# darioShar/DLPM

Measured on AMD Instinct MI355X. Metric: samples/sec at T=1000 (CIFAR-10 32x32, alpha=1.7), higher is better.
Workload: dtype f32 (1x1 / stride-2 convolutions: fp32 operands split exactly into 3 bf16 planes, bf16 MFMA products, fp32 accumulate)

## Files before the change

dlpm_amd/csrc/conv.h:

```cpp
#pragma once
#include "common.h"

namespace dlpm {

struct ConvLaunch {
    const float *src0 = nullptr, *src1 = nullptr;
    int C0 = 0, C1 = 0;
    int B = 0, Hin = 0, Win = 0, Hout = 0, Wout = 0;
    int ks = 1, stride = 1, ups = 0;
    const float *w = nullptr;
    const float *w_frag = nullptr;
    const float *w_wino = nullptr;
    const float *w_wino4 = nullptr;
    const float *w_wino4_n64 = nullptr, *w_wino4_n32 = nullptr;
    const float *w_wino4sp = nullptr;
    const void *w_split = nullptr;
    const float *w_small = nullptr;
    const float *w_taps = nullptr;
    const float *w_hfused = nullptr;
    const float *bias = nullptr;
    const float *coefA = nullptr, *coefB = nullptr;
    int act_silu = 0;
    const float *res0 = nullptr, *res1 = nullptr;
    int R0 = 0;
    float *out = nullptr;
    int Cout = 0;
    int in_nchw = 0, out_nchw = 0;
    int gen = 0;
    int64_t dispatch_B = 0;
    int gemm = 0;
    int ksplit = 0;
    float2 *stats_out = nullptr;
#ifdef DLPM_PHASE_TIMING
    unsigned long long *phase = nullptr;
#endif
};

bool igemm_supported(const ConvLaunch &c);

enum ConvFamily { CONV_HEAD_FUSED, CONV_HEAD_GEMM, CONV_HEAD, CONV_SPLIT, CONV_WINO4SP, CONV_WINO4, CONV_WINO, CONV_IGEMM, CONV_STEM, CONV_DIRECT };
struct ConvRoute {
    ConvFamily family = CONV_DIRECT;
    int bh = 0, bw = 0, nimg = 0;
    int nq = 0;
    int64_t grid = 0;
    int stats_px = 0;
    int ksplit = 1;
    int64_t scratch_floats = 0;
    char name[96] = "";
    bool head() const { return family <= CONV_HEAD; }
};
ConvRoute conv_route(const ConvLaunch &c);
struct HeadUpdate;
int launch_conv(const ConvLaunch &c, const HeadUpdate *hu, float *head_scratch, hipStream_t st);
int launch_conv_direct(const ConvLaunch &c, hipStream_t st);
int launch_conv_stem(const ConvLaunch &c, hipStream_t st);
struct HeadUpdate {
    float *x = nullptr;
    const float *z = nullptr;
// ... 21 lines not shown
int launch_conv_head_fused(const ConvLaunch &c, const HeadUpdate *hu, hipStream_t st);
bool wino_route(const ConvLaunch &c, ConvRoute *r);
int launch_conv_wino(const ConvLaunch &c, const ConvRoute &r, hipStream_t st);
int64_t wino_weight_floats(int Cout, int Cin);
int relayout_weight_wino(const float *oihw_dev, float *dst_dev, int Cout, int Cin, hipStream_t st);
bool wino4_enabled();
bool wino4_route(const ConvLaunch &c, ConvRoute *r);
int launch_conv_wino4(const ConvLaunch &c, const ConvRoute &r, hipStream_t st);
int64_t wino4_weight_floats(int Cout, int Cin);
int relayout_weight_wino4(const float *oihw_dev, float *dst_dev, int Cout, int Cin, hipStream_t st, int nq = 0);
bool wino4sp_enabled();
bool wino4sp_layer_ok(int Cout, int Cin, int Hlo, int Wlo);
int launch_conv_wino4sp(const ConvLaunch &c, const ConvRoute &r, hipStream_t st);
int64_t wino4sp_weight_floats(int Cout, int Cin);
int relayout_weight_wino4sp(const float *oihw_dev, float *dst_dev, int Cout, int Cin, hipStream_t st);
struct ResImgLaunch {
    const float *x0 = nullptr, *x1 = nullptr;
    int C0 = 0, C1 = 0, B = 0;
    int H = 32;
    const float2 *st0 = nullptr, *st1 = nullptr;
    int nt0 = 1, nt1 = 1;
    const float *coefA1 = nullptr, *coefB1 = nullptr;
    const float *gn1_w = nullptr, *gn1_b = nullptr, *gn2_w = nullptr, *gn2_b = nullptr;
    const float *w1 = nullptr, *b1 = nullptr;
    const float *w2 = nullptr, *b2 = nullptr;
    const float *emb = nullptr;
    int64_t emb_stride = 0;
    int emb_off = 0;
    const float *res = nullptr;
    float *hbuf = nullptr;
// ... 1 lines not shown
    float2 *stats_out = nullptr;
#ifdef DLPM_PHASE_TIMING
    unsigned long long *phase = nullptr;
#endif
};
bool res_img_ok(const ResImgLaunch &r);
int launch_resblock_img(const ResImgLaunch &r, hipStream_t st);

bool conv_split_ok(const ConvLaunch &c);
int launch_conv_split(const ConvLaunch &c, hipStream_t st);
int64_t split_weight_floats(int Cout, int Cin, int taps);
int relayout_weight_split(const float *oihw_dev, void *dst_dev, int Cout, int Cin, int taps, hipStream_t st);
constexpr int64_t NARROW_COPIES_MAX_BATCH = 512;
struct Conv3Layouts {
    bool frag = false, wino = false, wino4 = false, wino4sp = false;
    bool narrow = false;
};
bool wino4_narrow_copies_wanted(int Cout, int64_t dispatch_B);
Conv3Layouts conv3_layouts(const ConvLaunch &c);
int64_t splitk_partial_floats(const ConvLaunch &c, const ConvRoute &r);
int launch_conv_splitk(const ConvLaunch &c, const ConvRoute &r, float *part, hipStream_t st);
int launch_splitk_reduce(const float *part, int S, int64_t npix, int Cout, const float *bias, const float *res0, const float *res1, int R0,
                         float *out, hipStream_t st);
int relayout_weight(const float *oihw_dev, float *dst_dev, int Cout, int Cin, int ks, bool for_igemm, hipStream_t st);
int64_t frag_weight_floats(int Cout, int Cin);
int relayout_weight_frag(const float *oihw_dev, float *dst_dev, int Cout, int Cin, hipStream_t st);

int launch_gn_coeffs(const float *src0, const float *src1, int C0, int C1, int B, int HW, int groups,
                     const float *gamma, const float *beta, const float *ss, int64_t ss_stride, int64_t ss_offset,
                     float *coefA, float *coefB, hipStream_t st);
// ... 53 lines not shown
```

dlpm_amd/csrc/conv_igemm.hip:

```cpp
#include <cstdlib>

#include <algorithm>

#include "conv.h"
#include "igemm_epilogue.h"

namespace dlpm {
namespace {

constexpr int KC = 32;
constexpr int LDS_LD = 36;

template <int BN, int WAVES_M, int WAVES_N, int RM, int RN>
__device__ __forceinline__ void epilogue_rows(const ConvLaunch &p, floatx16 (&acc)[RM][RN], float *lds, int64_t m0, int n0,
                                              int64_t M, int tid, int wm, int wn, int l31, int kh) {
    constexpr int LD = BN + 4, PR = RM * 32, C4 = BN / 4, RG = 256 / C4;
    const int R1 = p.Cout - p.R0;
    const bool do_stats = p.stats_out != nullptr;
    float4 K = make_float4(0.f, 0.f, 0.f, 0.f), s1 = K, s2 = K;
    int cnt = 0;
    for (int ph = 0; ph < WAVES_M; ph++) {
        if (wm == ph) {
#pragma unroll
            for (int i = 0; i < RM; i++)
// ... 997 lines not shown
}

bool wino4_narrow_copies_wanted(int Cout, int64_t dispatch_B) {
    return Cout % 128 == 0 && dispatch_B > 0 && dispatch_B <= NARROW_COPIES_MAX_BATCH;
}

Conv3Layouts conv3_layouts(const ConvLaunch &c) {
    Conv3Layouts y;
    const int Cin = c.C0 + c.C1;
    const bool plain = !c.in_nchw && !c.out_nchw && c.stride == 1;
    if (!igemm_supported(c) || c.ks != 3 || Cin % 32 != 0) return y;
    y.frag = true;
    y.wino = plain && c.Cout % 64 == 0 && Cin % 16 == 0;
    y.wino4 = plain && wino4_enabled() && c.Cout % 32 == 0 && Cin % 8 == 0;
    y.wino4sp = y.wino4 && c.ups && wino4sp_layer_ok(c.Cout, Cin, c.Hin, c.Win);
    y.narrow = y.wino4 && wino4_narrow_copies_wanted(c.Cout, c.dispatch_B);
    return y;
}

ConvRoute conv_route(const ConvLaunch &c) {
    ConvRoute r;
    const int64_t hw = (int64_t)c.Hout * c.Wout;
    int th, nimg;
    const char *cls = nullptr;
    if (head_fused_ok(c)) {
        r.family = CONV_HEAD_FUSED;
    } else if (head_gemm_ok(c)) {
        r.family = CONV_HEAD_GEMM;
        r.scratch_floats = head_gemm_scratch_floats(c);
    } else if (head_conv_ok(c)) {
        r.family = CONV_HEAD;
    } else if (conv_split_ok(c)) {
        r.family = CONV_SPLIT;
        cls = c.ks == 1 ? "conv1x1_bf16x3" : "conv3x3_bf16x3";
        r.stats_px = (c.R0 & 3) ? 0 : hw % BM == 0 ? BM : hw == 64 ? 64 : 0;
    } else if (wino4_route(c, &r)) {
        cls = r.family == CONV_WINO4SP ? "conv3x3_wino4sp" : "conv3x3_wino4";
        if (r.family == CONV_WINO4 && r.nq != 128 && !(c.Cout == 32 && c.Hout == 32 && c.Wout == 32)) r.ksplit = ksplit_for(c, r.grid);
    } else if (!igemm_supported(c)) {
        r.family = conv_takes_stem(c) ? CONV_STEM : CONV_DIRECT;
        if (r.family == CONV_STEM && stem_stats_ok(c)) r.stats_px = 1024;
    } else if (wino_route(c, &r)) {
        cls = "conv3x3_wino";
        r.ksplit = ksplit_for(c, r.grid);
    } else {
        r.family = CONV_IGEMM;
        cls = c.ks == 3 ? (halo_ok(c, &th, &nimg) ? "conv3x3_halo" : "conv3x3_igemm") : "conv1x1_igemm";
        r.stats_px = (c.out_nchw || (c.Cout & 3) || (c.R0 & 3)) ? 0 : hw % BM == 0 ? BM : 0;
    }
    if (r.ksplit > 1) r.stats_px = 0;
    if (!cls) return r;
    if (prof_enabled() && prof_detail()) {
        const bool gemm = r.family == CONV_SPLIT || r.family == CONV_IGEMM;
// ... 107 lines not shown
```

dlpm_amd/csrc/conv_wino4.hip:

```cpp
#include <cstdlib>
#include <type_traits>

#include "conv.h"
#include "gn_stats.h"

namespace dlpm {
namespace {

typedef float floatx4 __attribute__((ext_vector_type(4)));

constexpr int F4_TILES = 16;
constexpr int F4_NQ = 128;
constexpr int F4_KC = 8;
constexpr int F4_RAWPIX = 576;
constexpr int F4_PRLD = F4_KC + 4;
constexpr int F4_NT = 512;
constexpr int F4_QNIT = (F4_RAWPIX * 2 + F4_NT - 1) / F4_NT;
constexpr int F4_RAWBUF = F4_RAWPIX * F4_PRLD + 16;
constexpr int F4_RAWPIX_N = 400;
constexpr int F4_RAWBUF_N = F4_RAWPIX_N * F4_PRLD + 16;
constexpr int f4_nq_of(int cout) { return cout % 128 == 0 ? 128 : cout % 64 == 0 ? 64 : 32; }
constexpr int F4_CFS = 16 * 2 * F4_KC;
constexpr int F4_VBUF = 36 * F4_TILES * F4_KC;
#ifndef F4_RING_DEPTH
// ... 1382 lines not shown
            F4_LDS_BARRIER();
            if (kh == 0 && lkv == 0) {
                const float2 a = part[chv], b = part[CO + chv];
                const float dd = b.x - a.x;
                p.stats_out[(int64_t)img * CO + chv] = make_float2(a.x + dd * 0.5f, a.y + b.y + dd * dd * 64.f);
            }
        }
    };
    if (kh == 0) epilogue(std::integral_constant<int, 0>());
    else epilogue(std::integral_constant<int, 2>());
    DLPM_PHASE(p, 10);
    DLPM_PHASE_FLUSH(p, 8);
#ifdef DLPM_PHASE_TIMING
    if (p.phase && tid == 0) atomicAdd(p.phase + 11, 1ull);
#endif
}

__global__ void k_relayout_weight_wino4(const float *oihw, float *dst, int Cout, int Cin, int nw) {
    const int nch = Cin / F4_KC;
    const int64_t total = (int64_t)Cout * Cin * 36;
    const int64_t i = (int64_t)blockIdx.x * blockDim.x + threadIdx.x;
    if (i >= total) return;
    const int e = (int)(i & 3);
    const int lane = (int)((i >> 2) & 63);
    int64_t r = i >> 8;
    const int pp = (int)(r % 18); r /= 18;
    const int chunk = (int)(r % nch); r /= nch;
    const int wave = (int)(r % nw);
    const int nt = (int)(r / nw);
    const int lk = lane >> 4, li = lane & 15;
// ... 109 lines not shown
    if (c.gen == DLPM_CONV_F2 || c.gen == DLPM_CONV_IGEMM) return false;
    if (!wino4_geometry_nq(c, nq, bh, bw, nimg)) return false;
    if (!c.w_wino || c.gen == DLPM_CONV_F4) return true;
    if (*nimg > 4) return false;
    if (c.dispatch_B <= 0) return true;
    return f4_mblocks(c.dispatch_B, c.Hout / 4, c.Wout / 4, *nimg) * (c.Cout / nq) >= 256;
}

static bool wino4_whole_image(const ConvLaunch &c) {
    static const int v = env_switch("DLPM_WINO4_IMG", 1);
    return v != 0 && c.Cout == 32 && !c.ups && c.Hout == 32 && c.Wout == 32 && (c.C0 + c.C1) <= 1024;
}

static int launch_conv_wino4_nq(const ConvLaunch &c, int nq, int bh, int bw, int nimg, hipStream_t st);

int launch_conv_wino4(const ConvLaunch &c, const ConvRoute &rt, hipStream_t st) {
    int bh, bw, nimg;
    if (rt.family != CONV_WINO4 || !wino4_geometry_nq(c, rt.nq, &bh, &bw, &nimg)) {
        set_error("launch_conv_wino4: unsupported shape");
        return DLPM_ERR_UNSUPPORTED;
    }
    const int nq = rt.nq;
    if (nq != f4_nq_of(c.Cout)) {
        ConvLaunch cn = c;
        cn.w_wino4 = nq == 64 ? c.w_wino4_n64 : c.w_wino4_n32;
        cn.w_wino4_n64 = cn.w_wino4_n32 = nullptr;
        cn.dispatch_B = 0;
        return launch_conv_wino4_nq(cn, nq, rt.bh, rt.bw, rt.nimg, st);
    }
    return launch_conv_wino4_nq(c, nq, rt.bh, rt.bw, rt.nimg, st);
}

// ... 103 lines not shown
    if (n * (4 * h + 1) * (4 * w + 1) > FS_RAWPIX) return false;
    *bh = h; *bw = w; *nimg = n;
    return true;
}
bool wino4sp_layer_ok(int Cout, int Cin, int Hlo, int Wlo) {
    int h, w, n;
    return wino4sp_enabled() && wino4sp_block(Cout, Cin, Hlo, Wlo, &h, &w, &n);
}

static bool wino4sp_geometry(const ConvLaunch &c, int *bh, int *bw, int *nimg) {
    if (!c.ups || !c.w_wino4sp || c.ks != 3 || c.stride != 1 || c.in_nchw || c.out_nchw) return false;
    if (c.Hout != 2 * c.Hin || c.Wout != 2 * c.Win || c.C0 % F4_KC != 0 || (c.R0 & 15) != 0 || c.ksplit > 1) return false;
    return wino4sp_block(c.Cout, c.C0 + c.C1, c.Hin, c.Win, bh, bw, nimg);
}

bool wino4_route(const ConvLaunch &c, ConvRoute *r) {
    const int nq = wino4_nq_for(c);
    int bh, bw, nimg;
    if (!wino4_preferred(c, nq, &bh, &bw, &nimg)) return false;
    r->family = CONV_WINO4;
    if (c.ups && c.w_wino4sp && wino4sp_enabled() && nq == F4_NQ && wino4sp_geometry(c, &bh, &bw, &nimg)) r->family = CONV_WINO4SP;
    else if (c.dispatch_B > 0) r->grid = f4_mblocks(c.dispatch_B, c.Hout / 4, c.Wout / 4, nimg) * (c.Cout / nq);
    r->bh = bh; r->bw = bw; r->nimg = nimg; r->nq = nq;
    r->stats_px = nimg == 1 ? 256 : (nimg == 4 && bh * bw == 4) ? 64 : 0;
    return true;
}

int launch_conv_wino4sp(const ConvLaunch &c, const ConvRoute &rt, hipStream_t st) {
    int bh, bw, nimg;
    if (rt.family != CONV_WINO4SP || !wino4sp_geometry(c, &bh, &bw, &nimg)) {
        set_error("launch_conv_wino4sp: unsupported shape");
// ... 23 lines not shown
```

dlpm_amd/csrc/unet.hip:

```cpp
#include <cmath>
#include <cstdlib>
#include <map>
#include <string>
#include <utility>
#include <vector>

#include "conv.h"
#include "../../include/dlpm_amd_chains.h"
#include "../../include/dlpm_amd_conv.h"

using namespace dlpm;

namespace {

struct Param {
    std::string key;
    int64_t numel = 0;
    float *dev = nullptr;
    bool set = false;
};

enum LayerKind { L_STEM, L_RES, L_ATTN, L_DOWN, L_UP };

struct ConvW {
    int p_w = -1, p_b = -1;
    int cout = 0, cin = 0, ks = 1;
    bool use_igemm = false;
    float *w_dev = nullptr;
    float *w_frag = nullptr;
    float *w_wino = nullptr;
    float *w_wino4 = nullptr;
    float *w_wino4_n64 = nullptr, *w_wino4_n32 = nullptr;
    float *w_wino4sp = nullptr;
    float *w_small = nullptr;
    float *w_taps = nullptr;
    float *w_split = nullptr;
    float *w_rs = nullptr;
    float *w_hfused = nullptr;
    bool owns = false;
};
constexpr float *ConvW::*OWNED_LAYOUTS[] = {&ConvW::w_frag, &ConvW::w_wino, &ConvW::w_wino4, &ConvW::w_wino4_n64, &ConvW::w_wino4_n32, &ConvW::w_wino4sp,
                                            &ConvW::w_small, &ConvW::w_taps, &ConvW::w_split, &ConvW::w_rs, &ConvW::w_hfused};
constexpr struct { int nq; float *ConvW::*copy; } NARROW_LAYOUTS[] = {{64, &ConvW::w_wino4_n64}, {32, &ConvW::w_wino4_n32}};

struct Layer {
    LayerKind kind;
    std::string pre;
    int cin = 0, cout = 0;
    int emb_off = 0;
    ConvW c1, c2, skip;
    bool has_skip = false;
    int p_gn1_w = -1, p_gn1_b = -1, p_gn2_w = -1, p_gn2_b = -1;
    int p_emb_w = -1, p_emb_b = -1;
};

struct Tensor4 {
// ... 192 lines not shown
                L.kind = L_UP; L.pre = pre + std::to_string(k++) + ".conv.";
                L.cin = L.cout = ch;
                L.c1 = u->conv(L.pre, ch, ch, 3);
                seq.push_back(L);
                ds /= 2;
            }
            u->out_blocks.push_back(seq);
        }
    }
    u->final_ch = ch;
    u->p_head_gn_w = u->add("out.0.weight", ch);
    u->p_head_gn_b = u->add("out.0.bias", ch);
    u->head = u->conv("out.2.", c.out_channels, mc, 3);
}

int prep_conv(dlpm_unet *u, ConvW &c, int C0, int boundary, int ups_lo = 0) {
    ConvLaunch probe;
    probe.C0 = C0; probe.C1 = c.cin - C0; probe.Cout = c.cout; probe.ks = c.ks;
    probe.in_nchw = boundary == 1; probe.out_nchw = boundary == 2;
    probe.stride = boundary == 4 ? 2 : 1; probe.ups = ups_lo > 0; probe.Hin = probe.Win = ups_lo;
    const Conv3Layouts lay = conv3_layouts(probe);
    c.use_igemm = igemm_supported(probe);
    const float *src = u->params[c.p_w].dev;
    if (c.use_igemm && c.ks == 1) {
        c.w_dev = const_cast<float *>(src);
        if (small_weight_ok(c.cout, c.cin, 1) && boundary == 0) {
            DLPM_HIP(hipMalloc(&c.w_rs, (size_t)small_weight_floats(c.cout, c.cin, 1) * sizeof(float)));
            int r = relayout_weight_small(src, c.w_rs, c.cout, c.cin, 1, nullptr);
            if (r != DLPM_OK) return r;
        }
        if (c.cout % 128 == 0 && c.cin % 32 == 0 && boundary == 0) {
            DLPM_HIP(hipMalloc(&c.w_split, (size_t)split_weight_floats(c.cout, c.cin, 1) * sizeof(float)));
            return relayout_weight_split(src, c.w_split, c.cout, c.cin, 1, nullptr);
        }
        return DLPM_OK;
// ... 26 lines not shown
        if (r != DLPM_OK) return r;
        if (lay.wino) {
            DLPM_HIP(hipMalloc(&c.w_wino, (size_t)wino_weight_floats(c.cout, c.cin) * sizeof(float)));
            r = relayout_weight_wino(src, c.w_wino, c.cout, c.cin, nullptr);
            if (r != DLPM_OK) return r;
        }
        if (lay.wino4) {
            DLPM_HIP(hipMalloc(&c.w_wino4, (size_t)wino4_weight_floats(c.cout, c.cin) * sizeof(float)));
            r = relayout_weight_wino4(src, c.w_wino4, c.cout, c.cin, nullptr);
            if (r != DLPM_OK) return r;
            if (lay.wino4sp) {
                DLPM_HIP(hipMalloc(&c.w_wino4sp, (size_t)wino4sp_weight_floats(c.cout, c.cin) * sizeof(float)));
                r = relayout_weight_wino4sp(src, c.w_wino4sp, c.cout, c.cin, nullptr);
                if (r != DLPM_OK) return r;
            }
        }
    }
    if (small_weight_ok(c.cout, c.cin, c.ks) && boundary == 0) {
        DLPM_HIP(hipMalloc(&c.w_rs, (size_t)small_weight_floats(c.cout, c.cin, c.ks) * sizeof(float)));
        int r = relayout_weight_small(src, c.w_rs, c.cout, c.cin, c.ks, nullptr);
        if (r != DLPM_OK) return r;
    }
    return relayout_weight(src, c.w_dev, c.cout, c.cin, c.ks, c.use_igemm, nullptr);
}

void attach_conv(const dlpm_unet *u, const ConvW &c, ConvLaunch &L) {
    policy_of(u, L);
    L.w = c.w_dev;
    L.w_frag = c.w_frag;
    L.w_wino = c.w_wino;
    L.w_wino4 = c.w_wino4;
    L.w_wino4_n64 = c.w_wino4_n64;
    L.w_wino4_n32 = c.w_wino4_n32;
    L.w_wino4sp = c.w_wino4sp;
    L.w_small = c.w_small;
    L.w_taps = c.w_taps;
    L.w_hfused = c.w_hfused;
    L.w_split = c.w_split;
    L.ks = c.ks;
    L.Cout = c.cout;
}

int run_conv(const dlpm_unet *u, const ConvW &c, ConvLaunch L, hipStream_t st, const HeadUpdate *hu = nullptr, float *head_scratch = nullptr) {
    attach_conv(u, c, L);
    return launch_conv(L, hu, head_scratch, st);
}

#define TRY(expr)                  \
    do {                           \
// ... 459 lines not shown
        if (!c.w_wino4 || c.cout % 128 != 0) return;
        const bool want = wino4_narrow_copies_wanted(c.cout, u->dispatch_B);
        for (auto &n : NARROW_LAYOUTS) {
            float *&dst = c.*n.copy;
            if (!want) free_dev(dst);
            if (!want || dst || rc != DLPM_OK) continue;
            if (hipMalloc(&dst, (size_t)wino4_weight_floats(c.cout, c.cin) * sizeof(float)) != hipSuccess) { dst = nullptr; rc = DLPM_ERR_HIP; set_error("narrow_wino4_copies: hipMalloc failed"); continue; }
            rc = relayout_weight_wino4(u->params[c.p_w].dev, dst, c.cout, c.cin, nullptr, n.nq);
        }
    });
    if (rc == DLPM_OK && hipDeviceSynchronize() != hipSuccess) { set_error("narrow_wino4_copies: synchronize failed"); rc = DLPM_ERR_HIP; }
    return rc;
}

static int prep_layer(dlpm_unet *u, Layer &L, int C0, int &res) {
    TRY(prep_conv(u, L.c1, C0, L.kind == L_STEM ? 1 : L.kind == L_DOWN ? 4 : 0, L.kind == L_UP ? res : 0));
    if (L.kind == L_DOWN) res = (res - 1) / 2 + 1;
    if (L.kind == L_UP) res *= 2;
    if (L.kind == L_RES || L.kind == L_ATTN) TRY(prep_conv(u, L.c2, L.c2.cin, 0));
    if (L.kind == L_RES && L.has_skip) TRY(prep_conv(u, L.skip, C0, 0));
    return DLPM_OK;
}

static int stack_emb(dlpm_unet *u, const Layer &L) {
    DLPM_HIP(hipMemcpy(u->embcat_w + (size_t)L.emb_off * u->ted, u->params[L.p_emb_w].dev, (size_t)2 * L.cout * u->ted * sizeof(float),
                       hipMemcpyDeviceToDevice));
    DLPM_HIP(hipMemcpy(u->embcat_b + L.emb_off, u->params[L.p_emb_b].dev, (size_t)2 * L.cout * sizeof(float), hipMemcpyDeviceToDevice));
    return DLPM_OK;
}

extern "C" int dlpm_unet_finalize(dlpm_unet *u) {
    DLPM_CHECK_ARG(u, "dlpm_unet_finalize: null handle");
    for (auto &p : u->params)
        if (!p.set) {
// ... 373 lines not shown
    const bool wino_shape = a->ksize == 3 && !L.w_split && !(a->force_direct & 2) && a->stride == 1 && !a->in_nchw && !a->out_nchw;
    if (ig && a->ksize == 3 && !L.w_split && Cin_ % 32 == 0 &&
        a->scratch_floats >= used + frag_weight_floats(a->Cout, Cin_)) {
        float *wf = scratch_dev + used;
        TRY(relayout_weight_frag(a->weight, wf, a->Cout, Cin_, st));
        L.w_frag = wf;
        used += frag_weight_floats(a->Cout, Cin_);
        if (wino_shape && a->Cout % 64 == 0 && a->scratch_floats >= used + wino_weight_floats(a->Cout, Cin_)) {
            float *ww = scratch_dev + used;
            TRY(relayout_weight_wino(a->weight, ww, a->Cout, Cin_, st));
            L.w_wino = ww;
            used += wino_weight_floats(a->Cout, Cin_);
        }
    }
    bool ask_f4 = false;
    if (wino_shape && (a->force_direct & (8 | 256)) && a->Cout % 32 == 0 && Cin_ % 8 == 0 &&
        a->scratch_floats >= used + wino4_weight_floats(a->Cout, Cin_)) {
        float *w4 = scratch_dev + used;
        TRY(relayout_weight_wino4(a->weight, w4, a->Cout, Cin_, st));
        L.w_wino4 = w4;
        L.w_wino = nullptr;
        used += wino4_weight_floats(a->Cout, Cin_);
        ask_f4 = true;
    }
    if ((a->force_direct & 256) && L.w_wino4 && a->Cout % 128 == 0 && a->scratch_floats >= used + wino4sp_weight_floats(a->Cout, Cin_))
        L.w_wino4sp = scratch_dev + used;
    const bool head_shape = a->ksize == 3 && a->C0 % 32 == 0 && a->C1 == 0;
    const int ask_head = !head_shape || a->Cout > 3 ? 0 : (a->force_direct & 64) ? 64 : (a->force_direct & 32);
    const int64_t taps_floats = (int64_t)head_taps_rows(a->Cout) * a->C0;
    float *small_dev = nullptr;
    if (ask_head == 64) {
        L.gemm = (a->force_direct & 128) ? DLPM_GEMM_F32 : DLPM_GEMM_AUTO;
        if (a->scratch_floats >= head_fused_weight_floats(a->C0)) L.w_hfused = scratch_dev;
    } else if (ask_head == 32) {
        if (a->scratch_floats >= taps_floats + head_gemm_scratch_floats(L)) L.w_taps = scratch_dev;
    } else if (!(a->force_direct & 7) && head_shape && a->Cout <= 4) {
        const int64_t front = (int64_t)a->Cout * a->C0 * 9 + frag_weight_floats(a->Cout, a->C0);
        if (a->scratch_floats >= front + 9 * a->C0 * 4) L.w_small = small_dev = scratch_dev + (a->scratch_floats - 9 * a->C0 * 4);
    }
    const ConvRoute R = conv_route(L);
    const bool f4 = R.family == CONV_WINO4 || R.family == CONV_WINO4SP;
    const bool direct = (a->force_direct & 1) && !R.head() && !f4;
    const int px = direct ? 0 : R.stats_px;
    const struct { bool asked, got; const char *msg; } asks[] = {
        {ask_f4, f4, "dlpm_conv2d_f32: force_direct bit 8 asks for the F(4x4,3x3) kernel, which does not take this geometry"},
        {(a->force_direct & 256) != 0, R.family == CONV_WINO4SP,
         "dlpm_conv2d_f32: force_direct bit 256 asks for the sub-pixel upsampling kernel, which does not take this geometry / scratch size"},
        {stats_out != nullptr, px > 0,
         "dlpm_conv2d_stats_f32: this launch emits no statistics (its kernel has no statistics epilogue, or its partials would not lie inside one image)"},
        {ask_head == 64, R.family == CONV_HEAD_FUSED, "dlpm_conv2d_f32: the one-pass head kernel does not take this shape / scratch size"},
        {ask_head == 32, R.family == CONV_HEAD_GEMM, "dlpm_conv2d_f32: the GEMM + gather head does not take this shape / scratch size"},
    };
    for (const auto &q : asks)
        if (q.asked && !q.got) {
            set_error("%s", q.msg);
            return DLPM_ERR_UNSUPPORTED;
        }
    if (stats_out) {
        L.stats_out = reinterpret_cast<float2 *>(stats_out);
        *stats_px = px;
    }
    if (R.family == CONV_WINO4SP) TRY(relayout_weight_wino4sp(a->weight, const_cast<float *>(L.w_wino4sp), a->Cout, Cin_, st));
    if (R.family == CONV_HEAD_FUSED) TRY(relayout_weight_head_fused(a->weight, scratch_dev, a->Cout, a->C0, st));
    if (R.family == CONV_HEAD_GEMM) TRY(relayout_weight_head_taps(a->weight, scratch_dev, a->Cout, a->C0, st));
    if (R.family == CONV_HEAD) TRY(relayout_weight_head(a->weight, small_dev, a->Cout, a->C0, st));
    if (direct) return launch_conv_direct(L, st);
    return launch_conv(L, nullptr, scratch_dev + taps_floats, st);
}

static int policy_launch(const dlpm_conv_args *a, int32_t generation, int64_t dispatch_batch, float *base, ConvLaunch *out,
                         Conv3Layouts *lay_out, int64_t *used_out) {
    DLPM_CHECK_ARG(a, "dlpm_conv_policy: null argument");
    DLPM_CHECK_ARG(generation >= DLPM_CONV_AUTO && generation <= DLPM_CONV_IGEMM, "dlpm_conv_policy: unknown generation %d", generation);
    DLPM_CHECK_ARG(dispatch_batch >= 0, "dlpm_conv_policy: negative dispatch batch");
    if (a->ksize != 3 || a->stride != 1 || a->in_nchw || a->out_nchw || a->Cout <= 4 || a->force_direct != 0) {
        set_error("dlpm_conv_policy: takes 3x3 stride-1 NHWC launches with Cout > 4 and force_direct = 0");
        return DLPM_ERR_UNSUPPORTED;
// ... 8 lines not shown
    L.dispatch_B = dispatch_batch;
    const Conv3Layouts lay = conv3_layouts(L);
    const int Cin = a->C0 + a->C1;
    int64_t used = 0;
    auto take = [&](bool has, int64_t nfloats) -> const float * {
        if (!has) return nullptr;
        const float *p = base + used;
        used += (nfloats + 63) / 64 * 64;
        return p;
    };
    L.w = take(true, (int64_t)a->Cout * Cin * 9);
    L.w_frag = take(lay.frag, lay.frag ? frag_weight_floats(a->Cout, Cin) : 0);
    L.w_wino = take(lay.wino, lay.wino ? wino_weight_floats(a->Cout, Cin) : 0);
    L.w_wino4 = take(lay.wino4, lay.wino4 ? wino4_weight_floats(a->Cout, Cin) : 0);
    L.w_wino4sp = take(lay.wino4sp, lay.wino4sp ? wino4sp_weight_floats(a->Cout, Cin) : 0);
    L.w_wino4_n64 = take(lay.narrow, lay.narrow ? wino4_weight_floats(a->Cout, Cin) : 0);
    L.w_wino4_n32 = take(lay.narrow, lay.narrow ? wino4_weight_floats(a->Cout, Cin) : 0);
    *out = L;
    *lay_out = lay;
    *used_out = used;
    return DLPM_OK;
}

static void policy_route_out(const ConvLaunch &L, const ConvRoute &R, int64_t used, dlpm_conv_route *r) {
    r->family = (int32_t)R.family;
    r->bh = R.bh; r->bw = R.bw; r->nimg = R.nimg; r->nq = R.nq; r->stats_px = R.stats_px; r->ksplit = R.ksplit;
    r->reserved = 0;
    r->grid = R.grid;
    r->scratch_floats = used;
    r->partial_floats = splitk_partial_floats(L, R);
// ... 31 lines not shown
                  (long long)(partial_dev ? partial_floats : 0));
        return DLPM_ERR_NOMEM;
    }
    if (stats_out && R.stats_px <= 0) {
        set_error("dlpm_conv_policy_f32: this launch emits no statistics (a split-K launch, or a kernel whose partials would not lie inside one image)");
        return DLPM_ERR_UNSUPPORTED;
    }
    hipStream_t st = as_stream(stream);
    const int Cin = a->C0 + a->C1;
    auto at = [](const float *p) { return const_cast<float *>(p); };
    TRY(relayout_weight(a->weight, at(L.w), a->Cout, Cin, 3, igemm_supported(L), st));
    if (lay.frag) TRY(relayout_weight_frag(a->weight, at(L.w_frag), a->Cout, Cin, st));
    if (lay.wino) TRY(relayout_weight_wino(a->weight, at(L.w_wino), a->Cout, Cin, st));
    if (lay.wino4) TRY(relayout_weight_wino4(a->weight, at(L.w_wino4), a->Cout, Cin, st));
    if (lay.wino4sp) TRY(relayout_weight_wino4sp(a->weight, at(L.w_wino4sp), a->Cout, Cin, st));
    if (lay.narrow) {
        TRY(relayout_weight_wino4(a->weight, at(L.w_wino4_n64), a->Cout, Cin, st, 64));
        TRY(relayout_weight_wino4(a->weight, at(L.w_wino4_n32), a->Cout, Cin, st, 32));
    }
    if (stats_out) {
        L.stats_out = reinterpret_cast<float2 *>(stats_out);
        *stats_px = R.stats_px;
    }
    if (route) policy_route_out(L, R, used, route);
    return launch_conv_splitk(L, R, partial_dev, st);
}

extern "C" int dlpm_groupnorm_coeffs_f32(const float *src0, const float *src1, int32_t C0, int32_t C1, int32_t B, int32_t HW,
                                         int32_t groups, const float *gamma, const float *beta, const float *ss,
                                         int64_t ss_stride, int64_t ss_offset, float *coefA, float *coefB,
// ... 145 lines not shown
```

Before: 27.68.

## Add one-tile F(4x4,3x3) Winograd kernel for 4x4 resolution layers

Adds a specialised Winograd F(4x4,3x3) kernel for 3x3 convolutions whose output is exactly 4x4, so each image is a single tile and padding is handled by zeroing the patch border. The kernel splits the input-channel reduction across two wave halves and reduces them through LDS, with a 64-channel output slice per workgroup. It is meant to replace the split-K or poorly filled generic wino4 launches at the lowest UNet resolution. It adds a separate weight layout copy, wiring through routing, prep, and the policy API, and is taken only when the grid is large enough.

```diff
diff --git a/dlpm_amd/csrc/conv.h b/dlpm_amd/csrc/conv.h
--- a/dlpm_amd/csrc/conv.h
+++ b/dlpm_amd/csrc/conv.h
@@ -14,6 +14,7 @@
     const float *w_wino4 = nullptr;
     const float *w_wino4_n64 = nullptr, *w_wino4_n32 = nullptr;
     const float *w_wino4sp = nullptr;
+    const float *w_wino4_one = nullptr;
     const void *w_split = nullptr;
     const float *w_small = nullptr;
     const float *w_taps = nullptr;
@@ -43,6 +44,7 @@
     ConvFamily family = CONV_DIRECT;
     int bh = 0, bw = 0, nimg = 0;
     int nq = 0;
+    int one = 0;
     int64_t grid = 0;
     int stats_px = 0;
     int ksplit = 1;
@@ -94,6 +96,8 @@
 int launch_conv_wino4sp(const ConvLaunch &c, const ConvRoute &r, hipStream_t st);
 int64_t wino4sp_weight_floats(int Cout, int Cin);
 int relayout_weight_wino4sp(const float *oihw_dev, float *dst_dev, int Cout, int Cin, hipStream_t st);
+bool wino4_one_enabled();
+bool wino4_one_layer_ok(int Cout, int C0, int C1, int H, int W);
 struct ResImgLaunch {
     const float *x0 = nullptr, *x1 = nullptr;
     int C0 = 0, C1 = 0, B = 0;
@@ -125,6 +129,7 @@
 constexpr int64_t NARROW_COPIES_MAX_BATCH = 512;
 struct Conv3Layouts {
     bool frag = false, wino = false, wino4 = false, wino4sp = false;
+    bool wino4_one = false;
     bool narrow = false;
 };
 bool wino4_narrow_copies_wanted(int Cout, int64_t dispatch_B);
diff --git a/dlpm_amd/csrc/conv_igemm.hip b/dlpm_amd/csrc/conv_igemm.hip
--- a/dlpm_amd/csrc/conv_igemm.hip
+++ b/dlpm_amd/csrc/conv_igemm.hip
@@ -1035,6 +1035,7 @@
     y.wino = plain && c.Cout % 64 == 0 && Cin % 16 == 0;
     y.wino4 = plain && wino4_enabled() && c.Cout % 32 == 0 && Cin % 8 == 0;
     y.wino4sp = y.wino4 && c.ups && wino4sp_layer_ok(c.Cout, Cin, c.Hin, c.Win);
+    y.wino4_one = y.wino4 && !c.ups && wino4_one_layer_ok(c.Cout, c.C0, c.C1, c.Hout, c.Wout);
     y.narrow = y.wino4 && wino4_narrow_copies_wanted(c.Cout, c.dispatch_B);
     return y;
 }
@@ -1056,8 +1057,8 @@
         cls = c.ks == 1 ? "conv1x1_bf16x3" : "conv3x3_bf16x3";
         r.stats_px = (c.R0 & 3) ? 0 : hw % BM == 0 ? BM : hw == 64 ? 64 : 0;
     } else if (wino4_route(c, &r)) {
-        cls = r.family == CONV_WINO4SP ? "conv3x3_wino4sp" : "conv3x3_wino4";
-        if (r.family == CONV_WINO4 && r.nq != 128 && !(c.Cout == 32 && c.Hout == 32 && c.Wout == 32)) r.ksplit = ksplit_for(c, r.grid);
+        cls = r.family == CONV_WINO4SP ? "conv3x3_wino4sp" : r.one ? "conv3x3_wino4_one" : "conv3x3_wino4";
+        if (r.family == CONV_WINO4 && !r.one && r.nq != 128 && !(c.Cout == 32 && c.Hout == 32 && c.Wout == 32)) r.ksplit = ksplit_for(c, r.grid);
     } else if (!igemm_supported(c)) {
         r.family = conv_takes_stem(c) ? CONV_STEM : CONV_DIRECT;
         if (r.family == CONV_STEM && stem_stats_ok(c)) r.stats_px = 1024;
diff --git a/dlpm_amd/csrc/conv_wino4.hip b/dlpm_amd/csrc/conv_wino4.hip
--- a/dlpm_amd/csrc/conv_wino4.hip
+++ b/dlpm_amd/csrc/conv_wino4.hip
@@ -1420,6 +1420,215 @@
 #ifdef DLPM_PHASE_TIMING
     if (p.phase && tid == 0) atomicAdd(p.phase + 11, 1ull);
 #endif
+}
+
+constexpr int F1_NQ = 64;
+constexpr int F1_IP = 16 * F4_KC + 4;
+constexpr int F1_RAWBUF = F4_TILES * F1_IP;
+constexpr int F1_HALF = 2 * F4_VBUF + 2 * F1_RAWBUF + 2 * F4_CFS;
+constexpr int F1_XCH = 4 * 36 * 64 * 4;
+constexpr int F1_LDS = F1_XCH > 2 * F1_HALF ? F1_XCH : 2 * F1_HALF;
+static_assert(F1_LDS * sizeof(float) <= 160 * 1024, "one workgroup's LDS");
+struct F4PatchOne {
+    const float *rb;
+    __device__ __forceinline__ float2 operator()(int i, int c) const {
+        if (i == 0 || i == 5 || c == 0 || c == 5) return make_float2(0.f, 0.f);
+        return *reinterpret_cast<const float2 *>(rb + ((i - 1) * 4 + (c - 1)) * F4_KC);
+    }
+};
+
+__global__ void __launch_bounds__(F4_NT, 1) k_conv3x3_wino4_one(ConvLaunch p_in) {
+    ConvLaunch p = p_in;
+    extern __shared__ __attribute__((aligned(16))) float wsm[];
+    const int tid = threadIdx.x, lane = tid & 63, wave = __builtin_amdgcn_readfirstlane(tid >> 6);
+    const int nw = wave & 3, kh = wave >> 2;
+    const int li = lane & 15, lk = lane >> 4;
+    float *V = wsm + kh * F1_HALF;
+    float *raw = V + 2 * F4_VBUF;
+    float *Cf = raw + 2 * F1_RAWBUF;
+    const int Cin = p.C0 + p.C1;
+    const int nch = Cin / (2 * F4_KC), kb = kh * nch;
+    const int ntn = p.Cout / F1_NQ, nmb = gridDim.x / ntn;
+    const int mb = blockIdx.x % nmb, n0 = (blockIdx.x / nmb) * F1_NQ;
+    const int img0 = mb * F4_TILES;
+
+    const int ht = tid & 255, squad = ht & 1;
+    int off[2], lo[2];
+#pragma unroll
+    for (int it = 0; it < 2; it++) {
+        const int pix = it * 128 + (ht >> 1);
+        const int img = pix >> 4, px = pix & 15;
+        off[it] = (img0 + img) >= p.B ? -1 : (img0 + img) * 16 + px;
+        lo[it] = (img * F1_IP + px * F4_KC + squad * 4) | ((img * 2 * F4_KC + squad * 4) << 16);
+    }
+    const bool has_coef = p.coefA != nullptr;
+    const int cf_img = ht >> 2, cf_isb = (ht >> 1) & 1;
+    const bool cf_mine = has_coef && ht < F4_TILES * 4;
+    const float *cf_base = has_coef ? ((cf_isb ? p.coefB : p.coefA) + (int64_t)min(img0 + cf_img, p.B - 1) * Cin + kb * F4_KC + squad * 4) : nullptr;
+    float4 xr[2], cfr = make_float4(0.f, 0.f, 0.f, 0.f);
+    auto load_raw_into = [&](float4 (&dst)[2], int chunk) {
+        const int c = (kb + chunk) * F4_KC + squad * 4;
+        const bool first = c < p.C0;
+        const float *sb = first ? p.src0 + c : p.src1 + (c - p.C0);
+        const int ld = first ? p.C0 : p.C1;
+#pragma unroll
+        for (int it = 0; it < 2; it++) dst[it] = *reinterpret_cast<const float4 *>(sb + (int64_t)max(off[it], 0) * ld);
+    };
+    auto load_coef = [&](int chunk) {
+        if (cf_mine) cfr = *reinterpret_cast<const float4 *>(cf_base + chunk * F4_KC);
+    };
+    auto store_coef = [&](int slot) {
+        if (cf_mine) *reinterpret_cast<float4 *>(Cf + slot * F4_CFS + cf_img * 2 * F4_KC + cf_isb * F4_KC + squad * 4) = cfr;
+    };
+    auto store_raw_item = [&](int slot, int it) {
+        float4 x = xr[it];
+        if (has_coef) {
+            const float4 ca = *reinterpret_cast<const float4 *>(Cf + slot * F4_CFS + (lo[it] >> 16));
+            const float4 cb = *reinterpret_cast<const float4 *>(Cf + slot * F4_CFS + (lo[it] >> 16) + F4_KC);
+            x = f4_affine4(x, ca, cb);
+        }
+        if (p.act_silu) x = f4_silu4(x);
+        if (off[it] < 0) x = make_float4(0.f, 0.f, 0.f, 0.f);
+        *reinterpret_cast<float4 *>(raw + slot * F1_RAWBUF + (lo[it] & 0xffff)) = x;
+    };
+    auto store_raw = [&](int slot) {
+#pragma unroll
+        for (int it = 0; it < 2; it++) store_raw_item(slot, it);
+    };
+
+    const int xrp = kh == 0 ? wave : 7 - wave;
+    const int rbase = (lane & 15) * F1_IP + (lane >> 4) * 2, vofs = lane * 4;
+    auto transform = [&](int slot) {
+        if (xrp < 3) f4_transform_rp(xrp, F4PatchOne{raw + slot * F1_RAWBUF + rbase}, V + slot * F4_VBUF + vofs, 4 * F4_TILES * 4);
+    };
+
+    const float4 *__restrict__ wp = reinterpret_cast<const float4 *>(p.w_wino4_one) + ((int64_t)((n0 / F1_NQ) * 4 + nw) * (Cin / F4_KC) + kb) * 18 * 64;
+    constexpr int AHEAD = F4_RING - 1;
+    float4 bq[F4_RING];
+    const float *asrc = V + lane * 4;
+
+    floatx4 acc[36];
+#pragma unroll
+    for (int q = 0; q < 36; q++)
+#pragma unroll
+        for (int r = 0; r < 4; r++) acc[q][r] = 0.f;
+
+    const int last = nch - 1;
+    float4 xr1[2], cfr1 = make_float4(0.f, 0.f, 0.f, 0.f), cfr2 = cfr1;
+    load_raw_into(xr, 0);
+    load_raw_into(xr1, min(1, last));
+    load_coef(0);
+    if (cf_mine) {
+        cfr1 = *reinterpret_cast<const float4 *>(cf_base + min(1, last) * F4_KC);
+        cfr2 = *reinterpret_cast<const float4 *>(cf_base + min(2, last) * F4_KC);
+    }
+#pragma unroll
+    for (int a = 0; a < F4_RING - 1; a++) bq[a] = wp[a * 64 + lane];
+    store_coef(0);
+    cfr = cfr1;
+    store_coef(1);
+    __syncthreads();
+    store_raw(0);
+#pragma unroll
+    for (int it = 0; it < 2; it++) xr[it] = xr1[it];
+    store_raw(1);
+    load_raw_into(xr, min(2, last));
+    __syncthreads();
+    transform(0);
+    cfr = cfr2;
+    store_coef(0);
+    __syncthreads();
+
+#pragma unroll 1
+    for (int chunk = 0; chunk < nch; chunk++) {
+        const int cur = chunk & 1, nxt = cur ^ 1;
+        const float *ab = asrc + cur * F4_VBUF;
+        load_coef(min(chunk + 3, last));
+        float4 aq[F4_AAHEAD + 1];
+#pragma unroll
+        for (int a = 0; a < F4_AAHEAD; a++) aq[a] = *reinterpret_cast<const float4 *>(ab + a * (4 * F4_TILES * 4));
+#pragma unroll
+        for (int pp = 0; pp < 18; pp++) {
+            if (pp >= F4_S0 && pp < F4_S0 + 2) store_raw_item(cur, pp - F4_S0);
+            if (pp == F4_S0 + 2) load_raw_into(xr, min(chunk + 3, last));
+            if (pp == F4_X) transform(nxt);
+            bq[(pp + AHEAD) % F4_RING] = wp[AHEAD * 64 + lane];
+            wp += 64;
+            if (pp + F4_AAHEAD < 18)
+                aq[(pp + F4_AAHEAD) % (F4_AAHEAD + 1)] = *reinterpret_cast<const float4 *>(ab + (pp + F4_AAHEAD) * (4 * F4_TILES * 4));
+            if (F4_PRIO) __builtin_amdgcn_s_setprio(0);
+            f4_mfma4(aq[pp % (F4_AAHEAD + 1)], bq[pp % F4_RING], acc[2 * pp], acc[2 * pp + 1]);
+            if (F4_PRIO) __builtin_amdgcn_s_setprio(1);
+        }
+        store_coef(nxt);
+        __syncthreads();
+    }
+    if (F4_PRIO) __builtin_amdgcn_s_setprio(0);
+
+    float4 *xb = reinterpret_cast<float4 *>(wsm) + nw * 36 * 64 + lane;
+    if (kh == 1) {
+#pragma unroll
+        for (int q = 0; q < 36; q++) xb[q * 64] = make_float4(acc[q][0], acc[q][1], acc[q][2], acc[q][3]);
+    }
+    __syncthreads();
+    if (kh == 1) return;
+#pragma unroll
+    for (int q0 = 0; q0 < 36; q0 += 6) {
+        float4 t[6];
+#pragma unroll
+        for (int q = 0; q < 6; q++) t[q] = xb[(q0 + q) * 64];
+#pragma unroll
+        for (int q = 0; q < 6; q++) {
+            acc[q0 + q][0] += t[q].x;
+            acc[q0 + q][1] += t[q].y;
+            acc[q0 + q][2] += t[q].z;
+            acc[q0 + q][3] += t[q].w;
+            asm volatile("" : "+v"(acc[q0 + q]) : : "memory");
+        }
+    }
+
+    const int ch = n0 + 16 * nw + li;
+    const float bias_v = p.bias ? p.bias[ch] : 0.f;
+    const bool has_res = p.res0 != nullptr;
+    const bool res_first = __builtin_amdgcn_readfirstlane(n0 + 16 * nw) < p.R0;
+    const float *res_u = has_res ? (res_first ? p.res0 : p.res1 - p.R0) : nullptr;
+    const int res_ld = res_first ? p.R0 : p.Cout - p.R0;
+    const int64_t pix0 = (int64_t)img0 * 16;
+    float *__restrict__ out_blk = p.out + pix0 * p.Cout;
+    const float *__restrict__ res_blk = has_res ? res_u + pix0 * res_ld : nullptr;
+    const bool do_stats = p.stats_out != nullptr;
+#pragma unroll
+    for (int r = 0; r < 4; r++) {
+        const int tile = 4 * lk + r;
+        const bool ok = img0 + tile < p.B;
+        float rs[16];
+        const uint32_t bo_o = (uint32_t)(tile * 16 * p.Cout + ch) * 4u, bo_r = (uint32_t)(tile * 16 * res_ld + ch) * 4u;
+        if (has_res && ok) {
+#pragma unroll
+            for (int k = 0; k < 16; k++) rs[k] = *reinterpret_cast<const float *>(reinterpret_cast<const char *>(res_blk + k * res_ld) + bo_r);
+        }
+        float Yt[16];
+        f4_out_tile(acc, r, Yt);
+        if (!ok) continue;
+        float K = 0.f, s1 = 0.f, s2 = 0.f;
+#pragma unroll
+        for (int k = 0; k < 16; k++) {
+            float v = Yt[k] + bias_v;
+            if (has_res) v += rs[k];
+            if (do_stats) {
+                if (k == 0) K = v;
+                const float dd = v - K;
+                s1 += dd;
+                s2 = fmaf(dd, dd, s2);
+            }
+            *reinterpret_cast<float *>(reinterpret_cast<char *>(out_blk + k * p.Cout) + bo_o) = v;
+        }
+        if (do_stats) {
+            float mean, M2;
+            f4_stats_lane<16>(K, s1, s2, mean, M2);
+            p.stats_out[(int64_t)(img0 + tile) * p.Cout + ch] = make_float2(mean, M2);
+        }
+    }
 }
 
 __global__ void k_relayout_weight_wino4(const float *oihw, float *dst, int Cout, int Cin, int nw) {
@@ -1559,8 +1768,11 @@
 
 static int launch_conv_wino4_nq(const ConvLaunch &c, int nq, int bh, int bw, int nimg, hipStream_t st);
 
+int launch_conv_wino4_one(const ConvLaunch &c, hipStream_t st);
+
 int launch_conv_wino4(const ConvLaunch &c, const ConvRoute &rt, hipStream_t st) {
     int bh, bw, nimg;
+    if (rt.family == CONV_WINO4 && rt.one) return launch_conv_wino4_one(c, st);
     if (rt.family != CONV_WINO4 || !wino4_geometry_nq(c, rt.nq, &bh, &bw, &nimg)) {
         set_error("launch_conv_wino4: unsupported shape");
         return DLPM_ERR_UNSUPPORTED;
@@ -1694,7 +1906,49 @@
     return wino4sp_block(c.Cout, c.C0 + c.C1, c.Hin, c.Win, bh, bw, nimg);
 }
 
+bool wino4_one_enabled() {
+    static const int v = env_switch("DLPM_WINO4_ONE", 1);
+    return v != 0 && wino4_enabled();
+}
+
+bool wino4_one_layer_ok(int Cout, int C0, int C1, int H, int W) {
+    return wino4_one_enabled() && H == 4 && W == 4 && Cout > 0 && Cout % F1_NQ == 0 && C0 > 0 && (C0 + C1) % (2 * F4_KC) == 0 && C0 % F4_KC == 0;
+}
+
+static bool wino4_one_geometry(const ConvLaunch &c) {
+    if (!c.w_wino4_one || c.ks != 3 || c.stride != 1 || c.ups || c.in_nchw || c.out_nchw || c.ksplit > 1) return false;
+    if ((c.R0 & 15) != 0) return false;
+    return c.Hout == 4 && c.Wout == 4 && c.Cout % F1_NQ == 0 && c.C0 > 0 && (c.C0 + c.C1) % (2 * F4_KC) == 0 && c.C0 % F4_KC == 0;
+}
+
+static bool wino4_one_taken(const ConvLaunch &c) {
+    if (c.gen != DLPM_CONV_AUTO && c.gen != DLPM_CONV_F4) return false;
+    if (!wino4_one_enabled() || !wino4_one_geometry(c)) return false;
+    if (c.dispatch_B <= 0) return c.gen == DLPM_CONV_F4;
+    return ceil_div(c.dispatch_B, (int64_t)F4_TILES) * (c.Cout / F1_NQ) >= 256;
+}
+
+int launch_conv_wino4_one(const ConvLaunch &c, hipStream_t st) {
+    if (!wino4_one_geometry(c)) {
+        set_error("launch_conv_wino4: the one-tile shape does not take this launch");
+        return DLPM_ERR_UNSUPPORTED;
+    }
+    const int r = ensure_dynamic_lds(reinterpret_cast<const void *>(&k_conv3x3_wino4_one), 160 * 1024);
+    if (r != DLPM_OK) return r;
+    k_conv3x3_wino4_one<<<(unsigned)(ceil_div((int64_t)c.B, (int64_t)F4_TILES) * (c.Cout / F1_NQ)), F4_NT, (size_t)F1_LDS * sizeof(float), st>>>(c);
+    DLPM_LAUNCH_CHECK();
+    return DLPM_OK;
+}
+
 bool wino4_route(const ConvLaunch &c, ConvRoute *r) {
+    if (wino4_one_taken(c)) {
+        r->family = CONV_WINO4;
+        r->one = 1;
+        r->bh = r->bw = 1; r->nimg = F4_TILES; r->nq = F1_NQ;
+        if (c.dispatch_B > 0) r->grid = ceil_div(c.dispatch_B, (int64_t)F4_TILES) * (c.Cout / F1_NQ);
+        r->stats_px = 16;
+        return true;
+    }
     const int nq = wino4_nq_for(c);
     int bh, bw, nimg;
     if (!wino4_preferred(c, nq, &bh, &bw, &nimg)) return false;
diff --git a/dlpm_amd/csrc/unet.hip b/dlpm_amd/csrc/unet.hip
--- a/dlpm_amd/csrc/unet.hip
+++ b/dlpm_amd/csrc/unet.hip
@@ -32,6 +32,7 @@
     float *w_wino4 = nullptr;
     float *w_wino4_n64 = nullptr, *w_wino4_n32 = nullptr;
     float *w_wino4sp = nullptr;
+    float *w_wino4_one = nullptr;
     float *w_small = nullptr;
     float *w_taps = nullptr;
     float *w_split = nullptr;
@@ -39,7 +40,7 @@
     float *w_hfused = nullptr;
     bool owns = false;
 };
-constexpr float *ConvW::*OWNED_LAYOUTS[] = {&ConvW::w_frag, &ConvW::w_wino, &ConvW::w_wino4, &ConvW::w_wino4_n64, &ConvW::w_wino4_n32, &ConvW::w_wino4sp,
+constexpr float *ConvW::*OWNED_LAYOUTS[] = {&ConvW::w_frag, &ConvW::w_wino, &ConvW::w_wino4, &ConvW::w_wino4_n64, &ConvW::w_wino4_n32, &ConvW::w_wino4sp, &ConvW::w_wino4_one,
                                             &ConvW::w_small, &ConvW::w_taps, &ConvW::w_split, &ConvW::w_rs, &ConvW::w_hfused};
 constexpr struct { int nq; float *ConvW::*copy; } NARROW_LAYOUTS[] = {{64, &ConvW::w_wino4_n64}, {32, &ConvW::w_wino4_n32}};
 
@@ -262,11 +263,12 @@
     u->head = u->conv("out.2.", c.out_channels, mc, 3);
 }
 
-int prep_conv(dlpm_unet *u, ConvW &c, int C0, int boundary, int ups_lo = 0) {
+int prep_conv(dlpm_unet *u, ConvW &c, int C0, int boundary, int ups_lo = 0, int res = 0) {
     ConvLaunch probe;
     probe.C0 = C0; probe.C1 = c.cin - C0; probe.Cout = c.cout; probe.ks = c.ks;
     probe.in_nchw = boundary == 1; probe.out_nchw = boundary == 2;
     probe.stride = boundary == 4 ? 2 : 1; probe.ups = ups_lo > 0; probe.Hin = probe.Win = ups_lo;
+    probe.Hout = probe.Wout = ups_lo > 0 ? 2 * ups_lo : res;
     const Conv3Layouts lay = conv3_layouts(probe);
     c.use_igemm = igemm_supported(probe);
     const float *src = u->params[c.p_w].dev;
@@ -323,6 +325,11 @@
                 r = relayout_weight_wino4sp(src, c.w_wino4sp, c.cout, c.cin, nullptr);
                 if (r != DLPM_OK) return r;
             }
+            if (lay.wino4_one) {
+                DLPM_HIP(hipMalloc(&c.w_wino4_one, (size_t)wino4_weight_floats(c.cout, c.cin) * sizeof(float)));
+                r = relayout_weight_wino4(src, c.w_wino4_one, c.cout, c.cin, nullptr, 64);
+                if (r != DLPM_OK) return r;
+            }
         }
     }
     if (small_weight_ok(c.cout, c.cin, c.ks) && boundary == 0) {
@@ -342,6 +349,7 @@
     L.w_wino4_n64 = c.w_wino4_n64;
     L.w_wino4_n32 = c.w_wino4_n32;
     L.w_wino4sp = c.w_wino4sp;
+    L.w_wino4_one = c.w_wino4_one;
     L.w_small = c.w_small;
     L.w_taps = c.w_taps;
     L.w_hfused = c.w_hfused;
@@ -831,10 +839,10 @@
 }
 
 static int prep_layer(dlpm_unet *u, Layer &L, int C0, int &res) {
-    TRY(prep_conv(u, L.c1, C0, L.kind == L_STEM ? 1 : L.kind == L_DOWN ? 4 : 0, L.kind == L_UP ? res : 0));
+    TRY(prep_conv(u, L.c1, C0, L.kind == L_STEM ? 1 : L.kind == L_DOWN ? 4 : 0, L.kind == L_UP ? res : 0, L.kind == L_RES ? res : 0));
     if (L.kind == L_DOWN) res = (res - 1) / 2 + 1;
     if (L.kind == L_UP) res *= 2;
-    if (L.kind == L_RES || L.kind == L_ATTN) TRY(prep_conv(u, L.c2, L.c2.cin, 0));
+    if (L.kind == L_RES || L.kind == L_ATTN) TRY(prep_conv(u, L.c2, L.c2.cin, 0, 0, L.kind == L_RES ? res : 0));
     if (L.kind == L_RES && L.has_skip) TRY(prep_conv(u, L.skip, C0, 0));
     return DLPM_OK;
 }
@@ -1238,7 +1246,7 @@
         }
     }
     bool ask_f4 = false;
-    if (wino_shape && (a->force_direct & (8 | 256)) && a->Cout % 32 == 0 && Cin_ % 8 == 0 &&
+    if (wino_shape && (a->force_direct & (8 | 256 | 512)) && a->Cout % 32 == 0 && Cin_ % 8 == 0 &&
         a->scratch_floats >= used + wino4_weight_floats(a->Cout, Cin_)) {
         float *w4 = scratch_dev + used;
         TRY(relayout_weight_wino4(a->weight, w4, a->Cout, Cin_, st));
@@ -1249,6 +1257,12 @@
     }
     if ((a->force_direct & 256) && L.w_wino4 && a->Cout % 128 == 0 && a->scratch_floats >= used + wino4sp_weight_floats(a->Cout, Cin_))
         L.w_wino4sp = scratch_dev + used;
+    const bool ask_one = (a->force_direct & 512) != 0;
+    if (ask_one && L.w_wino4 && !L.w_wino4sp && !a->upsample && wino4_one_layer_ok(a->Cout, a->C0, a->C1, a->Hout, a->Wout) &&
+        a->scratch_floats >= used + wino4_weight_floats(a->Cout, Cin_)) {
+        L.w_wino4_one = scratch_dev + used;
+        L.gen = DLPM_CONV_F4;
+    }
     const bool head_shape = a->ksize == 3 && a->C0 % 32 == 0 && a->C1 == 0;
     const int ask_head = !head_shape || a->Cout > 3 ? 0 : (a->force_direct & 64) ? 64 : (a->force_direct & 32);
     const int64_t taps_floats = (int64_t)head_taps_rows(a->Cout) * a->C0;
@@ -1270,6 +1284,8 @@
         {ask_f4, f4, "dlpm_conv2d_f32: force_direct bit 8 asks for the F(4x4,3x3) kernel, which does not take this geometry"},
         {(a->force_direct & 256) != 0, R.family == CONV_WINO4SP,
          "dlpm_conv2d_f32: force_direct bit 256 asks for the sub-pixel upsampling kernel, which does not take this geometry / scratch size"},
+        {ask_one, R.family == CONV_WINO4 && R.one,
+         "dlpm_conv2d_f32: force_direct bit 512 asks for the one-tile F(4x4) kernel, which does not take this geometry / scratch size"},
         {stats_out != nullptr, px > 0,
          "dlpm_conv2d_stats_f32: this launch emits no statistics (its kernel has no statistics epilogue, or its partials would not lie inside one image)"},
         {ask_head == 64, R.family == CONV_HEAD_FUSED, "dlpm_conv2d_f32: the one-pass head kernel does not take this shape / scratch size"},
@@ -1285,6 +1301,7 @@
         *stats_px = px;
     }
     if (R.family == CONV_WINO4SP) TRY(relayout_weight_wino4sp(a->weight, const_cast<float *>(L.w_wino4sp), a->Cout, Cin_, st));
+    if (R.family == CONV_WINO4 && R.one) TRY(relayout_weight_wino4(a->weight, const_cast<float *>(L.w_wino4_one), a->Cout, Cin_, st, 64));
     if (R.family == CONV_HEAD_FUSED) TRY(relayout_weight_head_fused(a->weight, scratch_dev, a->Cout, a->C0, st));
     if (R.family == CONV_HEAD_GEMM) TRY(relayout_weight_head_taps(a->weight, scratch_dev, a->Cout, a->C0, st));
     if (R.family == CONV_HEAD) TRY(relayout_weight_head(a->weight, small_dev, a->Cout, a->C0, st));
@@ -1323,6 +1340,7 @@
     L.w_wino = take(lay.wino, lay.wino ? wino_weight_floats(a->Cout, Cin) : 0);
     L.w_wino4 = take(lay.wino4, lay.wino4 ? wino4_weight_floats(a->Cout, Cin) : 0);
     L.w_wino4sp = take(lay.wino4sp, lay.wino4sp ? wino4sp_weight_floats(a->Cout, Cin) : 0);
+    L.w_wino4_one = take(lay.wino4_one, lay.wino4_one ? wino4_weight_floats(a->Cout, Cin) : 0);
     L.w_wino4_n64 = take(lay.narrow, lay.narrow ? wino4_weight_floats(a->Cout, Cin) : 0);
     L.w_wino4_n32 = take(lay.narrow, lay.narrow ? wino4_weight_floats(a->Cout, Cin) : 0);
     *out = L;
@@ -1384,6 +1402,7 @@
     if (lay.wino) TRY(relayout_weight_wino(a->weight, at(L.w_wino), a->Cout, Cin, st));
     if (lay.wino4) TRY(relayout_weight_wino4(a->weight, at(L.w_wino4), a->Cout, Cin, st));
     if (lay.wino4sp) TRY(relayout_weight_wino4sp(a->weight, at(L.w_wino4sp), a->Cout, Cin, st));
+    if (lay.wino4_one) TRY(relayout_weight_wino4(a->weight, at(L.w_wino4_one), a->Cout, Cin, st, 64));
     if (lay.narrow) {
         TRY(relayout_weight_wino4(a->weight, at(L.w_wino4_n64), a->Cout, Cin, st, 64));
         TRY(relayout_weight_wino4(a->weight, at(L.w_wino4_n32), a->Cout, Cin, st, 32));
```

New measurement: 28.00, median of 6. 1.1% higher.
